# nfmoore/databricks-kubernetes-mlops-poc

Hardware: NVIDIA B200
Metric: rows/sec at batch=65536x23f (higher is better)
Workload: dtype u16 ranks + f64acc

## Files before the change

databricks_kubernetes_mlops_poc_b200/_cabi.py:

```python

from __future__ import annotations

import ctypes as C
import os

import numpy as np

ROW_WORDS = 24
ROW_BYTES = 96
PACKED_ROW_WORDS = 16
PACKED_ROW_BYTES = 64
ROWS_WORDS24 = 0
ROWS_PACKED64 = 1
ROWS_RANKED = 2
SCORED_DTYPE = np.dtype([("proba1", np.float32), ("label", np.int32)])
SCORED_FULL_DTYPE = np.dtype(
    [("proba1", np.float64), ("label", np.int32), ("is_outlier", np.int32), ("outlier_score", np.float32), ("reserved", np.int32)]
)
MOMENT_VALUES = ROW_WORDS * 3

_PKG_DIR = os.path.dirname(os.path.abspath(__file__))
LIB_PATH = os.path.join(_PKG_DIR, "lib", "libb200forest.so")

WALK_NAMES = {0: "smem", 1: "global"}
# ... 4 lines not shown
    """An engine call failed; the reference convention is "any exception -> HTTP 500"."""


class Info(C.Structure):
    _fields_ = [
        ("device", C.c_int32),
        ("sm_count", C.c_int32),
        ("agg_mode", C.c_int32),
        ("walk_mode", C.c_int32),
        ("n_trees", C.c_int32),
        ("n_groups", C.c_int32),
        ("max_depth", C.c_int32),
        ("n_cat", C.c_int32),
        ("n_num", C.c_int32),
        ("smem_bytes", C.c_int32),
        ("block_threads", C.c_int32),
        ("rows_per_warp", C.c_int32),
        ("forest_bytes", C.c_int64),
        ("launches", C.c_int64),
        ("launches_tile", C.c_int64),
        ("tile_min_rows", C.c_int64),
        ("tile_ok", C.c_int32),
        ("tile_resident", C.c_int32),
        ("packed_ok", C.c_int32),
        ("tile_warps", C.c_int32),
        ("launches_split", C.c_int64),
        ("split_max_rows", C.c_int64),
        ("outlier_trees", C.c_int32),
        ("rank_ok", C.c_int32),
        ("launches_rank", C.c_int64),
        ("rank_smem_bytes", C.c_int32),
        ("rank_row_bytes", C.c_int32),
        ("rank_stream", C.c_int32),
        ("reserved2", C.c_int32),
    ]


class RankInfo(C.Structure):

    _fields_ = [
        ("ok", C.c_int32),
        ("row_bytes", C.c_int32),
        ("cat_bytes", C.c_int32),
        ("n_cat", C.c_int32),
        ("n_num", C.c_int32),
        ("depth", C.c_int32),
        ("n_trees", C.c_int32),
        ("layout_bytes", C.c_int32),
        ("cat_shift", C.c_int32 * 16),
        ("cat_bits", C.c_int32 * 16),
        ("n_thresholds", C.c_int32 * 24),
        ("n_pairs", C.c_int32),
        ("pairs", C.c_uint32 * 128),
        ("why", C.c_char * 160),
    ]


class StrColumn(C.Structure):

    _fields_ = [
        ("offsets", C.c_void_p),
        ("data", C.c_void_p),
        ("validity", C.c_void_p),
        ("offset", C.c_int64),
        ("data_bytes", C.c_int64),
        ("offsets_are_64", C.c_int32),
        ("reserved", C.c_int32),
# ... 183 lines not shown
```

databricks_kubernetes_mlops_poc_b200/csrc/b2f_api.cu:

```cuda
#include <cuda_runtime.h>
#include <dlfcn.h>
#include <nccl.h>
#include <stdarg.h>
#include <stddef.h>
#include <stdio.h>
#include <stdlib.h>
#include <string.h>

#include <algorithm>
#include <string>
#include <thread>
#include <new>
#include <vector>

#include "../../include/b2f.h"
#include "feature_moments.cuh"
#include "forest_blob.h"
#include "forest_predict.cuh"
#include "forest_predict_tile.cuh"
#include "forest_predict_rank.cuh"
#include "forest_rank.h"
#include "json_rows.h"
#include "row_encoder.h"

#define B2F_VERSION_STR "b200forest 0.1.0 (sm_100a)"
#define B2F_STREAMS 4
#define B2F_TICKETS 256
#define B2F_CHUNK_ROWS 16384
#define B2F_FLUSH_BYTES (256ull << 20)

static thread_local char g_err[512] = "";

static int set_err(int code, const char *fmt, ...) {
    va_list ap;
    va_start(ap, fmt);
    vsnprintf(g_err, sizeof(g_err), fmt, ap);
    va_end(ap);
    return code;
}
#define CUDA_TRY(expr)                                                                         \
    do {                                                                                       \
        cudaError_t e_ = (expr);                                                               \
        if (e_ != cudaSuccess)                                                                 \
            return set_err(B2F_ECUDA, "%s failed: %s (%s:%d)", #expr, cudaGetErrorString(e_), __FILE__, __LINE__); \
    } while (0)
// ... 68 lines not shown
};

struct b2f_model {
    int device = 0;
    int sm_count = 0;
    int max_smem_optin = 0;
    KParams kp;
    b2f_blob_header hdr;
    int walk_mode = B2F_WALK_GLOBAL;
    int smem_bytes = 0;
    int rows_per_warp_max = 2;
    int64_t chunk_rows = B2F_CHUNK_ROWS;
    std::vector<int64_t> chunk_plan;
    bool tile_ok = false;
    TParams tp;
    void *d_tile_layout = nullptr;
    TPiece *d_tile_pieces = nullptr;
    int tile_smem_bytes = 0;
    int tile_cwarps = B2F_TILE_WARPS_MIN;
    int64_t tile_min_rows = 32768;
    int64_t tile_layout_bytes = 0;
    int64_t launches_tile = 0;
    int64_t launches_split = 0;
    int64_t split_max_rows = 0;
    bool packed_ok = false;
    b2f_ranker rk;
    bool rank_ok = false;
    RParams rp;
    void *d_rank_layout = nullptr;
    int rank_smem_bytes = 0;
    int rank_u = 4;
    bool rank_stream = false;
    int64_t launches_rank = 0;
    void *d_blob = nullptr;
    int64_t forest_bytes = 0;
    b2f_model *outlier = nullptr;
    Slot slots[B2F_STREAMS];
    cudaStream_t compute = nullptr;
    TicketRec tickets[B2F_TICKETS];
    uint64_t next_ticket = 1;
    uint64_t next_slot = 0;
    void *d_mom_rows = nullptr;
    int64_t mom_cap_rows = 0;
    double *d_mom_partials = nullptr;
    int mom_blocks = 0;
    unsigned int *d_mom_ticket = nullptr;
    double *d_mom_out = nullptr;
    double *d_gather = nullptr;
    int gather_cap = 0;
    void *d_flush = nullptr;
    ncclComm_t comm = nullptr;
    int nranks = 0;
    int rank = 0;
    int64_t launches = 0;
};

static int validate_blob(const uint8_t *blob, size_t nbytes, b2f_blob_header *hdr_out) {
    if (!blob || nbytes < sizeof(b2f_blob_header)) return set_err(B2F_EINVAL, "forest blob too small (%zu bytes)", nbytes);
    b2f_blob_header h;
    memcpy(&h, blob, sizeof(h));
    if (memcmp(h.magic, B2F_BLOB_MAGIC, 8) != 0) return set_err(B2F_EINVAL, "forest blob: bad magic");
    if (h.version != B2F_BLOB_VERSION) return set_err(B2F_EINVAL, "forest blob: version %u, expected %u", h.version, B2F_BLOB_VERSION);
    if (h.header_bytes != B2F_BLOB_HEADER_BYTES || h.row_words != B2F_ROW_WORDS)
        return set_err(B2F_EINVAL, "forest blob: header_bytes=%u row_words=%u unsupported", h.header_bytes, h.row_words);
    if (h.agg_mode != B2F_AGG_RF_MEAN && h.agg_mode != B2F_AGG_GBDT_LOGISTIC && h.agg_mode != B2F_AGG_IFOREST)
        return set_err(B2F_EINVAL, "forest blob: unknown agg_mode %u", h.agg_mode);
    if (h.n_trees == 0 || h.n_trees > B2F_MAX_TREES) return set_err(B2F_EINVAL, "forest blob: n_trees=%u out of range [1,%d]", h.n_trees, B2F_MAX_TREES);
    if (h.n_groups != (h.n_trees + 31) / 32) return set_err(B2F_EINVAL, "forest blob: n_groups=%u inconsistent with n_trees=%u", h.n_groups, h.n_trees);
    if (h.n_cat + h.n_num > B2F_SENTINEL_WORD) return set_err(B2F_EINVAL, "forest blob: n_cat+n_num=%u exceeds %u", h.n_cat + h.n_num, B2F_SENTINEL_WORD);
    if (h.total_bytes != nbytes) return set_err(B2F_EINVAL, "forest blob: total_bytes=%llu but %zu given", (unsigned long long)h.total_bytes, nbytes);
    if (h.groups_off < sizeof(h) || h.groups_off + (uint64_t)h.n_groups * sizeof(b2f_blob_group) > nbytes)
        return set_err(B2F_EINVAL, "forest blob: group table out of bounds");
    if (h.chunks_off % 256 || h.chunks_off + h.chunks_bytes > nbytes) return set_err(B2F_EINVAL, "forest blob: chunk area out of bounds");
    if (!(h.denom > 0.0)) return set_err(B2F_EINVAL, "forest blob: denom must be positive");
    const b2f_blob_group *gt = reinterpret_cast<const b2f_blob_group *>(blob + h.groups_off);
    uint64_t expect_off = 0;
    for (uint32_t g = 0; g < h.n_groups; ++g) {
        b2f_blob_group gr;
        memcpy(&gr, &gt[g], sizeof(gr));
        if (gr.chunk_off != expect_off || gr.n_slots == 0 || gr.n_leaf_slots == 0 ||
            gr.chunk_bytes != (gr.n_slots + gr.n_leaf_slots) * 256u || (uint64_t)gr.chunk_off + gr.chunk_bytes > h.chunks_bytes ||
            gr.n_slots >= (1u << 24) || gr.n_leaf_slots >= (1u << 24) || gr.n_trees == 0 || gr.n_trees > 32)
            return set_err(B2F_EINVAL, "forest blob: group %u descriptor invalid", g);
        expect_off += gr.chunk_bytes;
        const uint32_t *N = reinterpret_cast<const uint32_t *>(blob + h.chunks_off + gr.chunk_off);
        for (uint32_t s = 0; s < gr.n_slots; ++s)
            for (uint32_t l = 0; l < 32; ++l) {
                const uint32_t t = N[(s * 32 + l) * 2], m = N[(s * 32 + l) * 2 + 1];
// ... 206 lines not shown
        if (s < 2) return false;
        *n_slots = s;
    }
    return true;
}

template <int D, int U, bool ST, typename OutT>
static cudaError_t rank_set_attr(int bytes) {
    return cudaFuncSetAttribute(k_forest_predict_rank<D, U, ST, OutT>, cudaFuncAttributeMaxDynamicSharedMemorySize, bytes);
}
template <int U, bool ST>
static cudaError_t rank_set_attr_all(int depth, int bytes) {
    cudaError_t e = cudaSuccess;
#define RK_ATTR(DD)                                                        \
    case DD:                                                               \
        e = rank_set_attr<DD, U, ST, float>(bytes);                        \
        if (e == cudaSuccess) e = rank_set_attr<DD, U, ST, double>(bytes); \
        break;
    switch (depth) {
        RK_ATTR(1) RK_ATTR(2) RK_ATTR(3) RK_ATTR(4) RK_ATTR(5) RK_ATTR(6) RK_ATTR(7) RK_ATTR(8)
        default: e = cudaErrorInvalidValue;
    }
#undef RK_ATTR
    return e;
}

static int rank_init(b2f_model *m, const uint8_t *blob) {
    m->rank_ok = false;
    ranker_build(&m->rk, blob, m->hdr);
    if (!m->rk.ok) return B2F_OK;
    const char *off = getenv("B2F_RANK");
    if (off && !strcmp(off, "0")) return B2F_OK;
    const int64_t layout_bytes = (int64_t)m->rk.layout.size();
    const int64_t base = B2F_RANK_XS_BYTES  + (int64_t)B2F_RANK_PARTIALS * 32 * 8 + 256;
    int max_tiles = (int)std::min<int64_t>(B2F_RANK_MAX_TILES, ((int64_t)m->max_smem_optin - base - layout_bytes) / B2F_RANK_XS_BYTES);
    if (const char *mt = getenv("B2F_RANK_MAX_TILES")) max_tiles = std::min(max_tiles, std::max(1, atoi(mt)));
    m->rank_stream = max_tiles < 8;
    if (const char *fs = getenv("B2F_RANK_STREAM")) m->rank_stream = atoi(fs) != 0;
    int64_t forest_smem = layout_bytes;
    m->rank_u = 4;
    if (const char *ru = getenv("B2F_RANK_U")) m->rank_u = atoi(ru) == 8 ? 8 : 4;
    if (m->rank_stream) {
        m->rank_u = 4;
        const int64_t piece = 8 * (int64_t)m->rk.tree_stride;
        forest_smem = 2 * piece;
        max_tiles = (int)std::min<int64_t>(B2F_RANK_MAX_TILES, ((int64_t)m->max_smem_optin - base - forest_smem) / B2F_RANK_XS_BYTES);
        if (max_tiles < 4 || piece % 16) return B2F_OK;
    }
    CUDA_TRY(cudaMalloc(&m->d_rank_layout, (size_t)layout_bytes));
    CUDA_TRY(cudaMemcpy(m->d_rank_layout, m->rk.layout.data(), (size_t)layout_bytes, cudaMemcpyHostToDevice));
    RParams &rp = m->rp;
    memset(&rp, 0, sizeof(rp));
    rp.layout = static_cast<const uint8_t *>(m->d_rank_layout);
    rp.layout_bytes = (uint32_t)layout_bytes;
    rp.tree_stride = m->rk.tree_stride;
    rp.n_trees_padded = m->rk.n_trees_padded;
    rp.depth = m->rk.depth;
    rp.agg_mode = (int)m->hdr.agg_mode;
    rp.n_cat = m->rk.n_cat;
    rp.n_num = m->rk.n_num;
    rp.row_bytes = m->rk.row_bytes;
    rp.cat_bytes = m->rk.cat_bytes;
    rp.max_tiles = max_tiles;
    rp.groups_per_piece = 2;
    rp.piece_bytes = 8u * m->rk.tree_stride;
    rp.n_pieces = m->rk.n_trees_padded / 8;
    rp.init_raw = m->hdr.init_raw;
    rp.denom = m->hdr.denom;
    rp.threshold = m->hdr.threshold;
    rp.mul_two = 2u;
    rp.mul_64k = 65536u;
    rp.add_64k = 65535u;
    rp.n_pairs = (int)m->rk.pairs.size();
    for (int j = 0; j < 16; ++j) {
        rp.cat_shift[j] = (uint8_t)m->rk.cat_shift[j];
        rp.cat_bits[j] = (uint8_t)m->rk.cat_bits[j];
        rp.cat_start[j] = 0;
        rp.cat_mask[j] = 0ull;
    }
    for (int i = rp.n_pairs - 1; i >= 0; --i) {
        const uint32_t j = m->rk.pairs[i] >> 16, c = m->rk.pairs[i] & 0xFFFFu;
        rp.cat_start[j] = (uint8_t)i;
        rp.cat_mask[j] |= 1ull << c;
    }
    m->rank_smem_bytes = (int)(B2F_RANK_XS_BYTES + (int64_t)max_tiles * B2F_RANK_XS_BYTES + (int64_t)B2F_RANK_PARTIALS * 32 * 8 + forest_smem);
    if (m->rank_stream)
        CUDA_TRY((rank_set_attr_all<4, true>(rp.depth, m->rank_smem_bytes)));
    else
        CUDA_TRY(m->rank_u == 8 ? (rank_set_attr_all<8, false>(rp.depth, m->rank_smem_bytes)) : (rank_set_attr_all<4, false>(rp.depth, m->rank_smem_bytes)));
    m->rank_ok = true;
    return B2F_OK;
}

static bool kn_env_is(const char *v) {
    const char *kn = getenv("B2F_KERNEL");
    return kn && !strcmp(kn, v);
}

static int model_init_cuda(b2f_model *m, const uint8_t *blob, size_t nbytes) {
    CUDA_TRY(cudaSetDevice(m->device));
    cudaDeviceProp prop;
    CUDA_TRY(cudaGetDeviceProperties(&prop, m->device));
    if (prop.major < 10)
        return set_err(B2F_ENODEV, "device %d is sm_%d%d; this library is built for sm_100a (B200) only", m->device, prop.major, prop.minor);
    m->sm_count = prop.multiProcessorCount;
    CUDA_TRY(cudaDeviceGetAttribute(&m->max_smem_optin, cudaDevAttrMaxSharedMemoryPerBlockOptin, m->device));

    CUDA_TRY(cudaMalloc(&m->d_blob, nbytes));
    CUDA_TRY(cudaMemcpy(m->d_blob, blob, nbytes, cudaMemcpyHostToDevice));
    m->forest_bytes = (int64_t)m->hdr.chunks_bytes;

    KParams &kp = m->kp;
    memset(&kp, 0, sizeof(kp));
    kp.chunks = static_cast<const uint8_t *>(m->d_blob) + m->hdr.chunks_off;
    kp.n_groups = (int)m->hdr.n_groups;
    kp.agg_mode = (int)m->hdr.agg_mode;
    kp.n_cat = (int)m->hdr.n_cat;
// ... 135 lines not shown
    if (ndev < 0) return nullptr;
    if (device < 0 || device >= ndev) {
        set_err(B2F_EINVAL, "device %d out of range (have %d)", device, ndev);
        return nullptr;
    }
    b2f_model *m = new (std::nothrow) b2f_model();
    if (!m) {
        set_err(B2F_ENOMEM, "out of host memory");
        return nullptr;
    }
    m->device = device;
    if (validate_blob(static_cast<const uint8_t *>(forest_blob), nbytes, &m->hdr) != B2F_OK ||
        model_init_cuda(m, static_cast<const uint8_t *>(forest_blob), nbytes) != B2F_OK) {
        char keep[sizeof(g_err)];
        memcpy(keep, g_err, sizeof(keep));
        b2f_model_destroy(m);
        memcpy(g_err, keep, sizeof(keep));
        return nullptr;
    }
    return m;
}

extern "C" void b2f_model_destroy(b2f_model *m) {
    if (!m) return;
    cudaSetDevice(m->device);
    cudaDeviceSynchronize();
    if (m->outlier) b2f_model_destroy(m->outlier);
    if (m->comm && g_nccl.CommDestroy) g_nccl.CommDestroy(m->comm);
    for (int s = 0; s < B2F_STREAMS; ++s) {
        Slot &sl = m->slots[s];
        if (sl.d_rows) cudaFree(sl.d_rows);
        if (sl.d_proba) cudaFree(sl.d_proba);
        if (sl.d_label) cudaFree(sl.d_label);
        if (sl.stream) cudaStreamDestroy(sl.stream);
    }
    for (auto &t : m->tickets)
        for (auto &e : t.ev)
            if (e) cudaEventDestroy(e);
    if (m->compute) cudaStreamDestroy(m->compute);
    if (m->d_blob) cudaFree(m->d_blob);
    if (m->d_tile_layout) cudaFree(m->d_tile_layout);
    if (m->d_tile_pieces) cudaFree(m->d_tile_pieces);
    if (m->d_rank_layout) cudaFree(m->d_rank_layout);
    if (m->d_mom_rows) cudaFree(m->d_mom_rows);
    if (m->d_mom_partials) cudaFree(m->d_mom_partials);
    if (m->d_mom_ticket) cudaFree(m->d_mom_ticket);
    if (m->d_mom_out) cudaFree(m->d_mom_out);
    if (m->d_gather) cudaFree(m->d_gather);
    if (m->d_flush) cudaFree(m->d_flush);
    delete m;
}

static int pick_rows_per_warp(const b2f_model *m, int64_t n) {
    int r = m->rows_per_warp_max;
    const int64_t warps = (int64_t)m->sm_count * B2F_PREDICT_WARPS;
    while (r > 1 && n / r < warps) r >>= 1;
    return r;
}

extern "C" int b2f_model_info(const b2f_model *m, b2f_info *out) {
    if (!m || !out) return set_err(B2F_EINVAL, "null argument");
    memset(out, 0, sizeof(*out));
    out->device = m->device;
    out->sm_count = m->sm_count;
    out->agg_mode = (int)m->hdr.agg_mode;
    out->walk_mode = m->walk_mode;
    out->n_trees = (int)m->hdr.n_trees;
    out->n_groups = (int)m->hdr.n_groups;
    out->max_depth = (int)m->hdr.max_depth;
    out->n_cat = (int)m->hdr.n_cat;
    out->n_num = (int)m->hdr.n_num;
    out->smem_bytes = m->smem_bytes;
    out->block_threads = B2F_PREDICT_THREADS;
    out->rows_per_warp = m->rows_per_warp_max;
    out->forest_bytes = m->forest_bytes;
    out->launches = m->launches + (m->outlier ? m->outlier->launches : 0);
    out->launches_tile = m->launches_tile + (m->outlier ? m->outlier->launches_tile : 0);
    out->tile_min_rows = m->tile_min_rows;
    out->tile_ok = m->tile_ok ? 1 : 0;
    out->tile_resident = (m->tile_ok && m->tp.n_pieces <= m->tp.n_slots) ? 1 : 0;
    out->packed_ok = m->packed_ok ? 1 : 0;
    out->tile_warps = m->tile_ok ? m->tile_cwarps : 0;
    out->launches_split = m->launches_split;
    out->split_max_rows = m->split_max_rows;
    out->outlier_trees = m->outlier ? (int)m->outlier->hdr.n_trees : 0;
    out->rank_ok = m->rank_ok ? 1 : 0;
    out->launches_rank = m->launches_rank;
    out->rank_smem_bytes = m->rank_ok ? m->rank_smem_bytes : 0;
    out->rank_row_bytes = m->rk.row_bytes;
    out->rank_stream = (m->rank_ok && m->rank_stream) ? 1 : 0;
    return B2F_OK;
}

extern "C" int b2f_model_rank_info(const b2f_model *m, b2f_rank_info *out) {
    if (!m || !out) return set_err(B2F_EINVAL, "null argument");
    fill_rank_info(&m->rk, m->rank_ok, out);
    if (m->rk.ok && !m->rank_ok) snprintf(out->why, sizeof(out->why), "the rank layout (%zu bytes) does not stay resident in shared memory", m->rk.layout.size());
    return B2F_OK;
}

extern "C" void *b2f_pinned_alloc(size_t nbytes) {
    void *p = nullptr;
    cudaError_t e = cudaHostAlloc(&p, nbytes ? nbytes : 1, cudaHostAllocPortable);
    if (e != cudaSuccess) {
        set_err(B2F_ENOMEM, "cudaHostAlloc(%zu) failed: %s", nbytes, cudaGetErrorString(e));
        return nullptr;
    }
    return p;
}
extern "C" void b2f_pinned_free(void *p) {
    if (p) cudaFreeHost(p);
}

template <int R, bool SMEM, bool PACKED, typename OutT>
static cudaError_t launch_one(const b2f_model *m, cudaStream_t st, const void *rows, int64_t n, void *proba, int32_t *label, int ostride) {
    const int64_t n_batches = (n + R - 1) / R;
    int64_t ctas = std::min<int64_t>(m->sm_count, n_batches);
    if (ctas < 1) ctas = 1;
    k_forest_predict<R, SMEM, PACKED, OutT><<<(unsigned)ctas, B2F_PREDICT_THREADS, SMEM ? m->smem_bytes : 0, st>>>(
        m->kp, static_cast<const uint32_t *>(rows), (long long)n, static_cast<OutT *>(proba), label, ostride);
    return cudaGetLastError();
}

template <bool PACKED, typename OutT>
static cudaError_t launch_tile(const b2f_model *m, cudaStream_t st, const void *rows, int64_t n, void *proba, int32_t *label, int ostride) {
    const int64_t n_tiles = (n + B2F_TILE_ROWS - 1) / B2F_TILE_ROWS;
    const unsigned ctas = (unsigned)std::max<int64_t>(1, std::min<int64_t>(m->sm_count, n_tiles));
    k_forest_predict_tile<PACKED, OutT><<<ctas, (unsigned)(m->tile_cwarps + 1) * 32u, m->tile_smem_bytes, st>>>(m->tp, static_cast<const uint32_t *>(rows), (long long)n,
                                                                                           static_cast<OutT *>(proba), label, ostride);
    return cudaGetLastError();
}

template <bool PACKED, typename OutT>
static cudaError_t launch_split(const b2f_model *m, cudaStream_t st, const void *rows, int64_t n, void *proba, int32_t *label, int ostride) {
    constexpr int R = 2;
    const unsigned ctas = (unsigned)((n + R - 1) / R);
    k_forest_predict_split<R, PACKED, OutT><<<ctas, 32u * (unsigned)m->kp.n_groups, 0, st>>>(m->kp, static_cast<const uint32_t *>(rows), (long long)n,
                                                                                            static_cast<OutT *>(proba), label, ostride);
    return cudaGetLastError();
}

template <int D, int U, bool ST, typename OutT>
static cudaError_t launch_rank_du(const b2f_model *m, cudaStream_t st, const void *rows, int64_t n, void *proba, int32_t *label, int ostride) {
    const int64_t n_tiles = (n + 31) / 32;
    cudaLaunchConfig_t cfg = {};
    cfg.gridDim = dim3((unsigned)std::max<int64_t>(1, std::min<int64_t>(m->sm_count, n_tiles)));
    cfg.blockDim = dim3(B2F_RANK_THREADS);
    cfg.dynamicSmemBytes = (size_t)m->rank_smem_bytes;
    cfg.stream = st;
    cudaLaunchAttribute attr[1];
    attr[0].id = cudaLaunchAttributeProgrammaticStreamSerialization;
    attr[0].val.programmaticStreamSerializationAllowed = 1;
    static const bool no_pdl = getenv("B2F_NO_PDL") != nullptr;
    cfg.attrs = attr;
    cfg.numAttrs = no_pdl ? 0 : 1;
    return cudaLaunchKernelEx(&cfg, k_forest_predict_rank<D, U, ST, OutT>, m->rp, static_cast<const uint8_t *>(rows), (long long)n,
                              static_cast<OutT *>(proba), label, ostride);
}
template <typename OutT>
static cudaError_t launch_rank(const b2f_model *m, cudaStream_t st, const void *rows, int64_t n, void *proba, int32_t *label, int ostride) {
#define RK_CASE(DD)                                                                                                  \
    case DD:                                                                                                         \
        if (m->rank_stream) return launch_rank_du<DD, 4, true, OutT>(m, st, rows, n, proba, label, ostride);          \
        return m->rank_u == 8 ? launch_rank_du<DD, 8, false, OutT>(m, st, rows, n, proba, label, ostride)             \
                              : launch_rank_du<DD, 4, false, OutT>(m, st, rows, n, proba, label, ostride);
    switch (m->rp.depth) {
        RK_CASE(1) RK_CASE(2) RK_CASE(3) RK_CASE(4) RK_CASE(5) RK_CASE(6) RK_CASE(7) RK_CASE(8)
    }
#undef RK_CASE
    return cudaErrorInvalidValue;
}

static size_t row_bytes_of(const b2f_model *m, int fmt) {
    return fmt == B2F_ROWS_RANKED ? (size_t)m->rk.row_bytes : (fmt == B2F_ROWS_PACKED64 ? B2F_PACKED_ROW_BYTES : B2F_ROW_BYTES);
}

static int check_row_format(const b2f_model *m, int fmt) {
    if (fmt == B2F_ROWS_WORDS24) return B2F_OK;
    if (fmt == B2F_ROWS_RANKED) {
        if (!m->rank_ok)
            return set_err(B2F_EINVAL, "B2F_ROWS_RANKED is not available for this model (%s)",
                           m->rk.ok ? "its rank layout fits neither shared memory nor the streaming ring" : m->rk.why);
        return B2F_OK;
    }
    if (fmt != B2F_ROWS_PACKED64) return set_err(B2F_EINVAL, "unknown row format %d", fmt);
    if (!m->packed_ok) return set_err(B2F_EINVAL, "this model's schema does not fit the packed 64-byte row (needs exactly 9 categoricals with <= 126 categories, <= 14 numerics)");
    return B2F_OK;
}

static int launch_predict(b2f_model *m, cudaStream_t st, const void *rows_dev, int64_t n, int fmt, void *proba_dev, int f64, int32_t *label_dev,
                          int ostride = 1) {
    if (n <= 0) return B2F_OK;
    const bool pk = fmt == B2F_ROWS_PACKED64;
    cudaError_t e;
    if (fmt == B2F_ROWS_RANKED) {
        e = f64 ? launch_rank<double>(m, st, rows_dev, n, proba_dev, label_dev, ostride) : launch_rank<float>(m, st, rows_dev, n, proba_dev, label_dev, ostride);
        if (e != cudaSuccess) return set_err(B2F_ECUDA, "k_forest_predict_rank launch failed: %s", cudaGetErrorString(e));
        m->launches++;
        m->launches_rank++;
        return B2F_OK;
    }
    if (m->tile_ok && n >= m->tile_min_rows) {
        e = pk ? (f64 ? launch_tile<true, double>(m, st, rows_dev, n, proba_dev, label_dev, ostride) : launch_tile<true, float>(m, st, rows_dev, n, proba_dev, label_dev, ostride))
               : (f64 ? launch_tile<false, double>(m, st, rows_dev, n, proba_dev, label_dev, ostride) : launch_tile<false, float>(m, st, rows_dev, n, proba_dev, label_dev, ostride));
        if (e != cudaSuccess) return set_err(B2F_ECUDA, "k_forest_predict_tile launch failed: %s", cudaGetErrorString(e));
        m->launches++;
        m->launches_tile++;
        return B2F_OK;
    }
    if (n <= m->split_max_rows) {
        e = pk ? (f64 ? launch_split<true, double>(m, st, rows_dev, n, proba_dev, label_dev, ostride) : launch_split<true, float>(m, st, rows_dev, n, proba_dev, label_dev, ostride))
               : (f64 ? launch_split<false, double>(m, st, rows_dev, n, proba_dev, label_dev, ostride) : launch_split<false, float>(m, st, rows_dev, n, proba_dev, label_dev, ostride));
        if (e != cudaSuccess) return set_err(B2F_ECUDA, "k_forest_predict_split launch failed: %s", cudaGetErrorString(e));
        m->launches++;
        m->launches_split++;
        return B2F_OK;
    }
    const int r = pick_rows_per_warp(m, n);
    const bool sm = m->walk_mode == B2F_WALK_SMEM;
#define DISPATCH_T(RR, SM, PK)                                                                                      \
    (f64 ? launch_one<RR, SM, PK, double>(m, st, rows_dev, n, proba_dev, label_dev, ostride)                         \
         : launch_one<RR, SM, PK, float>(m, st, rows_dev, n, proba_dev, label_dev, ostride))
#define DISPATCH(RR) (sm ? (pk ? DISPATCH_T(RR, true, true) : DISPATCH_T(RR, true, false)) : (pk ? DISPATCH_T(RR, false, true) : DISPATCH_T(RR, false, false)))
    if (r == 4)
        e = DISPATCH(4);
    else if (r == 2)
        e = DISPATCH(2);
    else
        e = DISPATCH(1);
#undef DISPATCH
#undef DISPATCH_T
    if (e != cudaSuccess) return set_err(B2F_ECUDA, "k_forest_predict launch failed: %s", cudaGetErrorString(e));
// ... 600 lines not shown
```

databricks_kubernetes_mlops_poc_b200/csrc/forest_predict_rank.cuh:

```cuda
#pragma once
#include <cuda_runtime.h>
#include <stdint.h>

#include "forest_predict.cuh"
#include "forest_predict_tile.cuh"

#define B2F_RANK_THREADS 1024
#define B2F_RANK_WARPS 32
#define B2F_RANK_MAX_TILES 16
#define B2F_RANK_XS_BYTES 8192
#define B2F_RANK_PARTIALS (B2F_RANK_WARPS + B2F_RANK_MAX_TILES)

struct RParams {
    const uint8_t *layout;
    uint32_t layout_bytes;
    uint32_t tree_stride;
    int32_t n_trees_padded;
    int32_t depth;
    int32_t agg_mode;
    int32_t n_cat;
    int32_t n_num;
    int32_t row_bytes;
    int32_t cat_bytes;
    int32_t max_tiles;
    int32_t n_pieces;
    int32_t groups_per_piece;
    uint32_t piece_bytes;
    double init_raw;
    double denom;
    double threshold;
    uint32_t mul_two;
    uint32_t mul_64k;
    uint32_t add_64k;
    int32_t n_pairs;
    uint8_t cat_shift[16];
    uint8_t cat_bits[16];
    uint8_t cat_start[16];
    unsigned long long cat_mask[16];
};

__device__ __forceinline__ void pdl_launch_dependents() { asm volatile("griddepcontrol.launch_dependents;" ::: "memory"); }
__device__ __forceinline__ void pdl_wait() { asm volatile("griddepcontrol.wait;" ::: "memory"); }

__device__ __forceinline__ uint32_t lds_u16(uint32_t a) {
    uint32_t v;
    asm volatile("{ .reg .u16 h; ld.shared.u16 h, [%1]; cvt.u32.u16 %0, h; }" : "=r"(v) : "r"(a));
    return v;
}

template <int D, int U>
__device__ __forceinline__ void rank_walk_group(uint32_t t0, uint32_t tree_stride, uint32_t xs_lane, uint32_t m2, uint32_t m64k, uint32_t a64k,
                                                double &acc) {
    uint32_t at[U], k4[U], k8[U];
#pragma unroll
    for (int u = 0; u < U; ++u) {
        at[u] = t0 + u * tree_stride;
        k4[u] = 4u - at[u];
        k8[u] = 8u - at[u];
    }
#pragma unroll
    for (int d = 0; d < D; ++d) {
#pragma unroll
        for (int u = 0; u < U; ++u) {
            const uint32_t nw = lds32(at[u]);
            const uint32_t v = lds_u16(xs_lane | (nw & 0x1F82u));
            const uint32_t x = v * m64k + a64k;
            at[u] = at[u] * m2 + (x >= nw ? k8[u] : k4[u]);
        }
    }
#pragma unroll
    for (int u = 0; u < U; ++u) acc += lds_f64(at[u] + at[u] + k4[u] + 4u - (4u << D));
}

template <int D, int U, bool STREAM, typename OutT>
__global__ void __launch_bounds__(B2F_RANK_THREADS, 1)
    k_forest_predict_rank(const __grid_constant__ RParams p, const uint8_t *__restrict__ rows, long long n, OutT *__restrict__ proba,
                          int32_t *__restrict__ label, int ostride) {
    extern __shared__ __align__(128) uint8_t smem[];
    __shared__ __align__(8) uint64_t forest_bar[2];

    const int tid = threadIdx.x;
    const int lane = tid & 31;
    const int warp = tid >> 5;

    pdl_launch_dependents();

    const uint32_t pad = (B2F_RANK_XS_BYTES - (smem_addr(smem) & (B2F_RANK_XS_BYTES - 1u))) & (B2F_RANK_XS_BYTES - 1u);
    uint8_t *xs_all = smem + pad;
    double *partial = reinterpret_cast<double *>(xs_all + (size_t)p.max_tiles * B2F_RANK_XS_BYTES);
    uint8_t *forest = reinterpret_cast<uint8_t *>(partial + B2F_RANK_PARTIALS * 32);

    if (tid == 0) {
        mbar_init(&forest_bar[0], 1);
        mbar_init(&forest_bar[1], 1);
        fence_mbar_init();
        fence_proxy_async();
        if constexpr (!STREAM) {
            mbar_arrive_expect_tx(&forest_bar[0], p.layout_bytes);
            for (uint32_t o = 0; o < p.layout_bytes; o += B2F_BULK_PIECE) {
                const uint32_t part = min(B2F_BULK_PIECE, p.layout_bytes - o);
                tma_bulk_g2s(forest + o, p.layout + o, part, &forest_bar[0]);
            }
        }
    }
    auto issue_piece = [&](uint32_t k) {
        const uint32_t slot = k & 1u, piece = k % (uint32_t)p.n_pieces;
        mbar_arrive_expect_tx(&forest_bar[slot], p.piece_bytes);
        tma_bulk_g2s(forest + slot * p.piece_bytes, p.layout + (size_t)piece * p.piece_bytes, p.piece_bytes, &forest_bar[slot]);
    };

    const uint32_t n_tiles = (uint32_t)((n + 31) >> 5);
    const uint32_t tq = n_tiles / gridDim.x, tr = n_tiles % gridDim.x;
    const uint32_t tile0 = blockIdx.x * tq + min(blockIdx.x, tr), cta_tiles = tq + (blockIdx.x < tr ? 1u : 0u);
    const uint32_t n_rounds = (cta_tiles + (uint32_t)p.max_tiles - 1u) / (uint32_t)p.max_tiles;
    const int groups = p.n_trees_padded / U;
    const uint32_t forest_addr = smem_addr(forest);
    const uint32_t xs_addr = smem_addr(xs_all);
    bool forest_ready = false;

    pdl_wait();

    for (uint32_t round = 0; round < n_rounds; ++round) {
        const uint32_t rt0 = cta_tiles * round / n_rounds, rt1 = cta_tiles * (round + 1u) / n_rounds;
        const int T = (int)(rt1 - rt0);
        const long long row0 = (long long)(tile0 + rt0) * 32;
        const int n_rows = (int)min((long long)T * 32, n - row0);
        if (round > 0) __syncthreads();

        {
            const int items = T * 32 * 2;
            const int num_words = (p.n_num + 1) >> 1, hot_words = (p.n_pairs + 1) >> 1;
            for (int it = tid; it < items; it += B2F_RANK_THREADS) {
                const int part = it >= T * 32 ? 1 : 0, r = it - part * (T * 32);
                const uint32_t col = xs_addr + (uint32_t)(r >> 5) * B2F_RANK_XS_BYTES + (uint32_t)(r & 31) * 4u;
                const bool live = r < n_rows;
                const uint8_t *row = rows + (size_t)(row0 + (live ? r : 0)) * p.row_bytes;
                if (part == 0) {
                    const uint32_t *q = reinterpret_cast<const uint32_t *>(row + p.cat_bytes);
                    for (int w = 0; w < num_words; ++w) {
                        uint32_t v = live ? __ldg(q + w) : 0u;
                        if (2 * w + 1 >= p.n_num) v &= 0xFFFFu;
                        asm volatile("st.shared.u32 [%0], %1;" ::"r"(col + (uint32_t)w * 128u), "r"(v) : "memory");
                    }
                } else {
                    const uint32_t hot = col + (uint32_t)num_words * 128u;
                    for (int w = 0; w < hot_words; ++w) asm volatile("st.shared.u32 [%0], %1;" ::"r"(hot + (uint32_t)w * 128u), "r"(0u) : "memory");
                    if (live) {
                        unsigned long long cw = __ldg(reinterpret_cast<const uint32_t *>(row));
                        if (p.cat_bytes == 8) cw |= (unsigned long long)__ldg(reinterpret_cast<const uint32_t *>(row) + 1) << 32;
                        for (int j = 0; j < p.n_cat; ++j) {
                            const uint32_t code1 = (uint32_t)(cw >> p.cat_shift[j]) & ((1u << p.cat_bits[j]) - 1u);
                            const unsigned long long m = p.cat_mask[j];
                            if (code1 != 0u && code1 <= 64u && ((m >> (code1 - 1u)) & 1ull)) {
                                const uint32_t slot = (uint32_t)p.cat_start[j] + (uint32_t)__popcll(m & ((1ull << (code1 - 1u)) - 1ull));
                                asm volatile("st.shared.u16 [%0], %1;" ::"r"(hot + (slot >> 1) * 128u + (slot & 1u) * 2u), "h"((uint16_t)1) : "memory");
                            }
                        }
                    }
                }
            }
        }
        if constexpr (STREAM) {
            if (tid == 0) {
                issue_piece(round * (uint32_t)p.n_pieces);
                if (p.n_pieces > 1) issue_piece(round * (uint32_t)p.n_pieces + 1u);
            }
        }
        __syncthreads();
        if constexpr (!STREAM) {
            if (!forest_ready) {
                mbar_wait(&forest_bar[0], 0);
                forest_ready = true;
            }
        }

        if constexpr (STREAM) {
            const int GP = p.groups_per_piece;
            const bool mine = warp < T * GP;
            const uint32_t xs_lane = xs_addr + (uint32_t)(warp / GP) * B2F_RANK_XS_BYTES + (uint32_t)lane * 4u;
            const uint32_t g_off = (uint32_t)(warp % GP) * U * p.tree_stride;
            double acc = 0.0;
            for (int piece = 0; piece < p.n_pieces; ++piece) {
                const uint32_t k = round * (uint32_t)p.n_pieces + (uint32_t)piece;
                mbar_wait(&forest_bar[k & 1u], (k >> 1) & 1u);
                if (mine) rank_walk_group<D, U>(forest_addr + (k & 1u) * p.piece_bytes + g_off, p.tree_stride, xs_lane, p.mul_two, p.mul_64k, p.add_64k, acc);
                __syncthreads();
                if (tid == 0 && piece + 2 < p.n_pieces) issue_piece(k + 2u);
            }
            if (mine) partial[warp * 32 + lane] = acc;
            __syncthreads();
            for (int r = tid; r < n_rows; r += B2F_RANK_THREADS) {
                const int t = r >> 5, ln = r & 31;
                double s = p.agg_mode == B2F_AGG_GBDT_LOGISTIC ? p.init_raw : 0.0;
                for (int g = 0; g < GP; ++g) s += partial[(t * GP + g) * 32 + ln];
                double p1;
                int lab;
                aggregate(p.agg_mode, p.agg_mode == B2F_AGG_GBDT_LOGISTIC ? 0.0 : p.init_raw, p.denom, p.threshold, s, p1, lab);
                const long long row = row0 + r;
                if (proba) proba[row * ostride_p(ostride)] = (OutT)p1;
                if (label) label[row * ostride_l(ostride)] = lab;
            }
            continue;
        }

        {
            const int units = T * groups;
            int u = warp * units / B2F_RANK_WARPS;
            const int u_end = (warp + 1) * units / B2F_RANK_WARPS;
            while (u < u_end) {
                const int t = u / groups;
                const int g_end = min(groups, u_end - t * groups);
                const uint32_t xs_lane = xs_addr + (uint32_t)t * B2F_RANK_XS_BYTES + (uint32_t)lane * 4u;
                double acc = 0.0;
                for (int g = u - t * groups; g < g_end; ++g)
                    rank_walk_group<D, U>(forest_addr + (uint32_t)(g * U) * p.tree_stride, p.tree_stride, xs_lane, p.mul_two, p.mul_64k, p.add_64k, acc);
                partial[(warp + t) * 32 + lane] = acc;
                u = t * groups + g_end;
            }
        }
        __syncthreads();

        for (int r = tid; r < n_rows; r += B2F_RANK_THREADS) {
            const int t = r >> 5, ln = r & 31;
            const int units = T * groups;
            const int w_first = (int)(((uint32_t)(t * groups + 1) * B2F_RANK_WARPS + (uint32_t)units - 1u) / (uint32_t)units) - 1;
            const int w_last = (int)(((uint32_t)((t + 1) * groups) * B2F_RANK_WARPS + (uint32_t)units - 1u) / (uint32_t)units) - 1;
            double s = p.agg_mode == B2F_AGG_GBDT_LOGISTIC ? p.init_raw : 0.0;
            for (int w = w_first; w <= w_last; ++w)
                if ((w + 1) * units / B2F_RANK_WARPS > w * units / B2F_RANK_WARPS) s += partial[(w + t) * 32 + ln];
            double p1;
            int lab;
            aggregate(p.agg_mode, p.agg_mode == B2F_AGG_GBDT_LOGISTIC ? 0.0 : p.init_raw, p.denom, p.threshold, s, p1, lab);
            const long long row = row0 + r;
            if (proba) proba[row * ostride_p(ostride)] = (OutT)p1;
            if (label) label[row * ostride_l(ostride)] = lab;
        }
    }
    if constexpr (!STREAM) {
        if (!forest_ready) mbar_wait(&forest_bar[0], 0);
    }
}
```

include/b2f.h:

```cpp
#ifndef B2F_H
#define B2F_H

#include <stddef.h>
#include <stdint.h>

#ifdef __cplusplus
extern "C" {
#endif

#define B2F_ROW_WORDS 24
#define B2F_ROW_BYTES 96
#define B2F_PACKED_ROW_BYTES 64
#define B2F_MAX_TREES 1024
#define B2F_MOMENT_WORDS 3

#define B2F_ROWS_WORDS24 0
#define B2F_ROWS_PACKED64 1

#define B2F_ROWS_RANKED 2

#define B2F_OK 0
#define B2F_EINVAL (-1)
#define B2F_ECUDA (-2)
#define B2F_ENODEV (-3)
// ... 25 lines not shown
    float outlier_score;
    int32_t reserved;
} b2f_scored_full;

typedef struct b2f_info {
    int32_t device;
    int32_t sm_count;
    int32_t agg_mode;
    int32_t walk_mode;
    int32_t n_trees;
    int32_t n_groups;
    int32_t max_depth;
    int32_t n_cat;
    int32_t n_num;
    int32_t smem_bytes;
    int32_t block_threads;
    int32_t rows_per_warp;
    int64_t forest_bytes;
    int64_t launches;
    int64_t launches_tile;
    int64_t tile_min_rows;
    int32_t tile_ok;
    int32_t tile_resident;
    int32_t packed_ok;
    int32_t tile_warps;
    int64_t launches_split;
    int64_t split_max_rows;
    int32_t outlier_trees;
    int32_t rank_ok;
    int64_t launches_rank;
    int32_t rank_smem_bytes;
    int32_t rank_row_bytes;
    int32_t rank_stream;
    int32_t reserved2;
} b2f_info;

const char *b2f_version(void);
const char *b2f_last_error(void);
int b2f_device_count(void);

int b2f_blob_validate(const void *forest_blob, size_t nbytes);
b2f_model *b2f_model_create(const void *forest_blob, size_t nbytes, int device);
void b2f_model_destroy(b2f_model *m);
int b2f_model_info(const b2f_model *m, b2f_info *out);

typedef struct b2f_rank_info {
    int32_t ok;
    int32_t row_bytes;
    int32_t cat_bytes;
    int32_t n_cat, n_num;
    int32_t depth;
    int32_t n_trees;
    int32_t layout_bytes;
    int32_t cat_shift[16];
    int32_t cat_bits[16];
    int32_t n_thresholds[24];
    int32_t n_pairs;
    uint32_t pairs[128];
    char why[160];
} b2f_rank_info;
typedef struct b2f_ranker b2f_ranker;
b2f_ranker *b2f_ranker_create(const void *forest_blob, size_t nbytes);
void b2f_ranker_destroy(b2f_ranker *r);
int b2f_ranker_info(const b2f_ranker *r, b2f_rank_info *out);
const float *b2f_ranker_thresholds(const b2f_ranker *r, int k, int32_t *count);
const void *b2f_ranker_layout(const b2f_ranker *r, int64_t *nbytes);
int b2f_ranker_rank_rows(const b2f_ranker *r, const void *rows, int64_t n, int row_format, void *ranked_out, int threads);
// ... 129 lines not shown
```

Before: 3.722 billion.

## Defer PDL wait past tree walk, add packed head records, track output hazards

Moves the griddepcontrol.wait in the ranked forest kernel from before row staging to after the tree walk, so a dependent launch can stage rows and walk trees while the previous kernel finishes. To keep this safe, the host records each stream's recent output ranges and turns PDL off when the new input rows overlap prior outputs. It also adds a packed per-group head table with the root and level-1 nodes of each tree, read with vector shared loads, to cut scattered loads in the first two levels. A compile-time tracing hook is included. The trade-offs are extra shared memory for the head table, which can lower max_tiles, and a host mutex plus hash map lookup on every launch.

```diff
diff --git a/databricks_kubernetes_mlops_poc_b200/_cabi.py b/databricks_kubernetes_mlops_poc_b200/_cabi.py
--- a/databricks_kubernetes_mlops_poc_b200/_cabi.py
+++ b/databricks_kubernetes_mlops_poc_b200/_cabi.py
@@ -60,7 +60,7 @@
         ("rank_smem_bytes", C.c_int32),
         ("rank_row_bytes", C.c_int32),
         ("rank_stream", C.c_int32),
-        ("reserved2", C.c_int32),
+        ("rank_last_pdl", C.c_int32),
     ]
 
 
diff --git a/databricks_kubernetes_mlops_poc_b200/csrc/b2f_api.cu b/databricks_kubernetes_mlops_poc_b200/csrc/b2f_api.cu
--- a/databricks_kubernetes_mlops_poc_b200/csrc/b2f_api.cu
+++ b/databricks_kubernetes_mlops_poc_b200/csrc/b2f_api.cu
@@ -8,9 +8,12 @@
 #include <string.h>
 
 #include <algorithm>
+#include <deque>
+#include <mutex>
 #include <string>
 #include <thread>
 #include <new>
+#include <unordered_map>
 #include <vector>
 
 #include "../../include/b2f.h"
@@ -145,6 +148,10 @@
     int rank_u = 4;
     bool rank_stream = false;
     int64_t launches_rank = 0;
+    bool rank_last_pdl = false;
+#ifdef B2F_RANK_TRACE
+    unsigned long long *d_rank_trace = nullptr;
+#endif
     void *d_blob = nullptr;
     int64_t forest_bytes = 0;
     b2f_model *outlier = nullptr;
@@ -167,6 +174,40 @@
     int rank = 0;
     int64_t launches = 0;
 };
+
+struct RankWrites {
+    uintptr_t p0, p1, l0, l1;
+};
+static std::mutex g_rank_writes_mu;
+static std::unordered_map<cudaStream_t, std::deque<RankWrites>> g_rank_writes;
+
+static bool rank_launch_pdl(cudaStream_t st, int sm_count, const void *rows, size_t rows_bytes, const void *proba, size_t psz, const int32_t *label,
+                            int64_t n, int ostride) {
+    static const bool no_pdl = getenv("B2F_NO_PDL") != nullptr;
+    const int64_t ps = ostride & 0xffff, ls = (ostride >> 16) ? (ostride >> 16) : ps;
+    RankWrites w;
+    w.p0 = reinterpret_cast<uintptr_t>(proba);
+    w.p1 = proba ? w.p0 + (size_t)((n - 1) * ps + 1) * psz : w.p0;
+    w.l0 = reinterpret_cast<uintptr_t>(label);
+    w.l1 = label ? w.l0 + (size_t)((n - 1) * ls + 1) * sizeof(int32_t) : w.l0;
+    const uintptr_t r0 = reinterpret_cast<uintptr_t>(rows), r1 = r0 + rows_bytes;
+    std::lock_guard<std::mutex> lk(g_rank_writes_mu);
+    std::deque<RankWrites> &chain = g_rank_writes[st];
+    bool pdl = !no_pdl;
+    for (const RankWrites &c : chain)
+        if ((c.p0 < r1 && r0 < c.p1) || (c.l0 < r1 && r0 < c.l1)) {
+            pdl = false;
+            break;
+        }
+    if (!pdl) chain.clear();
+    chain.push_back(w);
+    while (chain.size() > 2 * (size_t)sm_count + 1) chain.pop_front();
+    return pdl;
+}
+static void rank_forget_stream(cudaStream_t st) {
+    std::lock_guard<std::mutex> lk(g_rank_writes_mu);
+    g_rank_writes.erase(st);
+}
 
 static int validate_blob(const uint8_t *blob, size_t nbytes, b2f_blob_header *hdr_out) {
     if (!blob || nbytes < sizeof(b2f_blob_header)) return set_err(B2F_EINVAL, "forest blob too small (%zu bytes)", nbytes);
@@ -439,29 +480,47 @@
     const char *off = getenv("B2F_RANK");
     if (off && !strcmp(off, "0")) return B2F_OK;
     const int64_t layout_bytes = (int64_t)m->rk.layout.size();
+    const int64_t head_bytes = (int64_t)m->rk.n_trees_padded * 12;
     const int64_t base = B2F_RANK_XS_BYTES  + (int64_t)B2F_RANK_PARTIALS * 32 * 8 + 256;
-    int max_tiles = (int)std::min<int64_t>(B2F_RANK_MAX_TILES, ((int64_t)m->max_smem_optin - base - layout_bytes) / B2F_RANK_XS_BYTES);
+    int max_tiles = (int)std::min<int64_t>(B2F_RANK_MAX_TILES, ((int64_t)m->max_smem_optin - base - layout_bytes - head_bytes) / B2F_RANK_XS_BYTES);
     if (const char *mt = getenv("B2F_RANK_MAX_TILES")) max_tiles = std::min(max_tiles, std::max(1, atoi(mt)));
     m->rank_stream = max_tiles < 8;
     if (const char *fs = getenv("B2F_RANK_STREAM")) m->rank_stream = atoi(fs) != 0;
-    int64_t forest_smem = layout_bytes;
+    int64_t forest_smem = layout_bytes + head_bytes;
     m->rank_u = 4;
     if (const char *ru = getenv("B2F_RANK_U")) m->rank_u = atoi(ru) == 8 ? 8 : 4;
+    std::vector<uint8_t> dev_layout(m->rk.layout);
     if (m->rank_stream) {
         m->rank_u = 4;
         const int64_t piece = 8 * (int64_t)m->rk.tree_stride;
         forest_smem = 2 * piece;
         max_tiles = (int)std::min<int64_t>(B2F_RANK_MAX_TILES, ((int64_t)m->max_smem_optin - base - forest_smem) / B2F_RANK_XS_BYTES);
         if (max_tiles < 4 || piece % 16) return B2F_OK;
-    }
-    CUDA_TRY(cudaMalloc(&m->d_rank_layout, (size_t)layout_bytes));
-    CUDA_TRY(cudaMemcpy(m->d_rank_layout, m->rk.layout.data(), (size_t)layout_bytes, cudaMemcpyHostToDevice));
+    } else {
+        const int U = m->rank_u, n_nodes = 1 << m->rk.depth;
+        std::vector<uint32_t> head((size_t)head_bytes / 4, 0u);
+        for (int t = 0; t < m->rk.n_trees_padded; ++t) {
+            const uint32_t *nodes = reinterpret_cast<const uint32_t *>(m->rk.layout.data() + (size_t)t * m->rk.tree_stride);
+            uint32_t *g = head.data() + (size_t)(t / U) * 3 * U;
+            g[t % U] = nodes[0];
+            if (n_nodes > 2) {
+                g[U + 2 * (t % U)] = nodes[1];
+                g[U + 2 * (t % U) + 1] = nodes[2];
+            }
+        }
+        dev_layout.resize((size_t)(layout_bytes + head_bytes));
+        memcpy(dev_layout.data() + layout_bytes, head.data(), (size_t)head_bytes);
+    }
+    CUDA_TRY(cudaMalloc(&m->d_rank_layout, dev_layout.size()));
+    CUDA_TRY(cudaMemcpy(m->d_rank_layout, dev_layout.data(), dev_layout.size(), cudaMemcpyHostToDevice));
     RParams &rp = m->rp;
     memset(&rp, 0, sizeof(rp));
     rp.layout = static_cast<const uint8_t *>(m->d_rank_layout);
-    rp.layout_bytes = (uint32_t)layout_bytes;
+    rp.layout_bytes = (uint32_t)dev_layout.size();
     rp.tree_stride = m->rk.tree_stride;
     rp.n_trees_padded = m->rk.n_trees_padded;
+    rp.n_groups = (m->rk.n_trees + m->rank_u - 1) / m->rank_u;
+    rp.head_off = (uint32_t)layout_bytes;
     rp.depth = m->rk.depth;
     rp.agg_mode = (int)m->hdr.agg_mode;
     rp.n_cat = m->rk.n_cat;
@@ -490,6 +549,11 @@
         rp.cat_start[j] = (uint8_t)i;
         rp.cat_mask[j] |= 1ull << c;
     }
+#ifdef B2F_RANK_TRACE
+    const size_t trace_bytes = (size_t)B2F_RANK_TRACE_LAUNCHES * m->sm_count * B2F_RANK_TRACE_WORDS * sizeof(unsigned long long);
+    CUDA_TRY(cudaMalloc(&m->d_rank_trace, trace_bytes));
+    CUDA_TRY(cudaMemset(m->d_rank_trace, 0, trace_bytes));
+#endif
     m->rank_smem_bytes = (int)(B2F_RANK_XS_BYTES + (int64_t)max_tiles * B2F_RANK_XS_BYTES + (int64_t)B2F_RANK_PARTIALS * 32 * 8 + forest_smem);
     if (m->rank_stream)
         CUDA_TRY((rank_set_attr_all<4, true>(rp.depth, m->rank_smem_bytes)));
@@ -691,16 +755,25 @@
         if (sl.d_rows) cudaFree(sl.d_rows);
         if (sl.d_proba) cudaFree(sl.d_proba);
         if (sl.d_label) cudaFree(sl.d_label);
-        if (sl.stream) cudaStreamDestroy(sl.stream);
+        if (sl.stream) {
+            rank_forget_stream(sl.stream);
+            cudaStreamDestroy(sl.stream);
+        }
     }
     for (auto &t : m->tickets)
         for (auto &e : t.ev)
             if (e) cudaEventDestroy(e);
-    if (m->compute) cudaStreamDestroy(m->compute);
+    if (m->compute) {
+        rank_forget_stream(m->compute);
+        cudaStreamDestroy(m->compute);
+    }
     if (m->d_blob) cudaFree(m->d_blob);
     if (m->d_tile_layout) cudaFree(m->d_tile_layout);
     if (m->d_tile_pieces) cudaFree(m->d_tile_pieces);
     if (m->d_rank_layout) cudaFree(m->d_rank_layout);
+#ifdef B2F_RANK_TRACE
+    if (m->d_rank_trace) cudaFree(m->d_rank_trace);
+#endif
     if (m->d_mom_rows) cudaFree(m->d_mom_rows);
     if (m->d_mom_partials) cudaFree(m->d_mom_partials);
     if (m->d_mom_ticket) cudaFree(m->d_mom_ticket);
@@ -748,6 +821,7 @@
     out->rank_smem_bytes = m->rank_ok ? m->rank_smem_bytes : 0;
     out->rank_row_bytes = m->rk.row_bytes;
     out->rank_stream = (m->rank_ok && m->rank_stream) ? 1 : 0;
+    out->rank_last_pdl = m->rank_last_pdl ? 1 : 0;
     return B2F_OK;
 }
 
@@ -800,7 +874,7 @@
 }
 
 template <int D, int U, bool ST, typename OutT>
-static cudaError_t launch_rank_du(const b2f_model *m, cudaStream_t st, const void *rows, int64_t n, void *proba, int32_t *label, int ostride) {
+static cudaError_t launch_rank_du(const b2f_model *m, cudaStream_t st, const void *rows, int64_t n, void *proba, int32_t *label, int ostride, bool pdl) {
     const int64_t n_tiles = (n + 31) / 32;
     cudaLaunchConfig_t cfg = {};
     cfg.gridDim = dim3((unsigned)std::max<int64_t>(1, std::min<int64_t>(m->sm_count, n_tiles)));
@@ -810,19 +884,37 @@
     cudaLaunchAttribute attr[1];
     attr[0].id = cudaLaunchAttributeProgrammaticStreamSerialization;
     attr[0].val.programmaticStreamSerializationAllowed = 1;
-    static const bool no_pdl = getenv("B2F_NO_PDL") != nullptr;
     cfg.attrs = attr;
-    cfg.numAttrs = no_pdl ? 0 : 1;
-    return cudaLaunchKernelEx(&cfg, k_forest_predict_rank<D, U, ST, OutT>, m->rp, static_cast<const uint8_t *>(rows), (long long)n,
+    cfg.numAttrs = pdl ? 1 : 0;
+#ifdef B2F_RANK_TRACE
+    RParams rp = m->rp;
+    rp.trace = m->d_rank_trace + (size_t)(m->launches_rank % B2F_RANK_TRACE_LAUNCHES) * m->sm_count * B2F_RANK_TRACE_WORDS;
+#else
+    const RParams &rp = m->rp;
+#endif
+    return cudaLaunchKernelEx(&cfg, k_forest_predict_rank<D, U, ST, OutT>, rp, static_cast<const uint8_t *>(rows), (long long)n,
                               static_cast<OutT *>(proba), label, ostride);
 }
+
+#ifdef B2F_RANK_TRACE
+extern "C" int64_t b2f_rank_trace_read(b2f_model *m, unsigned long long *out, int32_t *launch_slots, int32_t *ctas_per_launch) {
+    if (!m || !out || !m->d_rank_trace) return -1;
+    if (cudaSetDevice(m->device) != cudaSuccess || cudaDeviceSynchronize() != cudaSuccess) return -1;
+    if (cudaMemcpy(out, m->d_rank_trace, (size_t)B2F_RANK_TRACE_LAUNCHES * m->sm_count * B2F_RANK_TRACE_WORDS * sizeof(unsigned long long),
+                   cudaMemcpyDeviceToHost) != cudaSuccess)
+        return -1;
+    *launch_slots = B2F_RANK_TRACE_LAUNCHES;
+    *ctas_per_launch = m->sm_count;
+    return m->launches_rank;
+}
+#endif
 template <typename OutT>
-static cudaError_t launch_rank(const b2f_model *m, cudaStream_t st, const void *rows, int64_t n, void *proba, int32_t *label, int ostride) {
+static cudaError_t launch_rank(const b2f_model *m, cudaStream_t st, const void *rows, int64_t n, void *proba, int32_t *label, int ostride, bool pdl) {
 #define RK_CASE(DD)                                                                                                  \
     case DD:                                                                                                         \
-        if (m->rank_stream) return launch_rank_du<DD, 4, true, OutT>(m, st, rows, n, proba, label, ostride);          \
-        return m->rank_u == 8 ? launch_rank_du<DD, 8, false, OutT>(m, st, rows, n, proba, label, ostride)             \
-                              : launch_rank_du<DD, 4, false, OutT>(m, st, rows, n, proba, label, ostride);
+        if (m->rank_stream) return launch_rank_du<DD, 4, true, OutT>(m, st, rows, n, proba, label, ostride, pdl);     \
+        return m->rank_u == 8 ? launch_rank_du<DD, 8, false, OutT>(m, st, rows, n, proba, label, ostride, pdl)        \
+                              : launch_rank_du<DD, 4, false, OutT>(m, st, rows, n, proba, label, ostride, pdl);
     switch (m->rp.depth) {
         RK_CASE(1) RK_CASE(2) RK_CASE(3) RK_CASE(4) RK_CASE(5) RK_CASE(6) RK_CASE(7) RK_CASE(8)
     }
@@ -853,10 +945,13 @@
     const bool pk = fmt == B2F_ROWS_PACKED64;
     cudaError_t e;
     if (fmt == B2F_ROWS_RANKED) {
-        e = f64 ? launch_rank<double>(m, st, rows_dev, n, proba_dev, label_dev, ostride) : launch_rank<float>(m, st, rows_dev, n, proba_dev, label_dev, ostride);
+        const bool pdl = rank_launch_pdl(st, m->sm_count, rows_dev, (size_t)n * (size_t)m->rk.row_bytes, proba_dev, f64 ? sizeof(double) : sizeof(float), label_dev, n, ostride);
+        e = f64 ? launch_rank<double>(m, st, rows_dev, n, proba_dev, label_dev, ostride, pdl)
+                : launch_rank<float>(m, st, rows_dev, n, proba_dev, label_dev, ostride, pdl);
         if (e != cudaSuccess) return set_err(B2F_ECUDA, "k_forest_predict_rank launch failed: %s", cudaGetErrorString(e));
         m->launches++;
         m->launches_rank++;
+        m->rank_last_pdl = pdl;
         return B2F_OK;
     }
     if (m->tile_ok && n >= m->tile_min_rows) {
diff --git a/databricks_kubernetes_mlops_poc_b200/csrc/forest_predict_rank.cuh b/databricks_kubernetes_mlops_poc_b200/csrc/forest_predict_rank.cuh
--- a/databricks_kubernetes_mlops_poc_b200/csrc/forest_predict_rank.cuh
+++ b/databricks_kubernetes_mlops_poc_b200/csrc/forest_predict_rank.cuh
@@ -16,6 +16,8 @@
     uint32_t layout_bytes;
     uint32_t tree_stride;
     int32_t n_trees_padded;
+    int32_t n_groups;
+    uint32_t head_off;
     int32_t depth;
     int32_t agg_mode;
     int32_t n_cat;
@@ -37,7 +39,35 @@
     uint8_t cat_bits[16];
     uint8_t cat_start[16];
     unsigned long long cat_mask[16];
+#ifdef B2F_RANK_TRACE
+    unsigned long long *trace;
+#endif
 };
+
+#define B2F_RANK_TRACE_WORDS 8
+#define B2F_RANK_TRACE_LAUNCHES 256
+enum { RT_SMID, RT_ENTRY, RT_FOREST, RT_WAIT, RT_STAGED, RT_WALKED, RT_EXIT };
+#ifdef B2F_RANK_TRACE
+__device__ __forceinline__ unsigned long long rank_trace_now() {
+    unsigned long long t;
+    asm volatile("mov.u64 %0, %%globaltimer;" : "=l"(t));
+    return t;
+}
+__device__ __forceinline__ unsigned long long rank_trace_smid() {
+    uint32_t s;
+    asm volatile("mov.u32 %0, %%smid;" : "=r"(s));
+    return s;
+}
+#define RANK_TRACE(i)                                                                                                       \
+    do {                                                                                                                    \
+        if (threadIdx.x == 0)                                                                                               \
+            p.trace[(size_t)blockIdx.x * B2F_RANK_TRACE_WORDS + (i)] = (i) == RT_SMID ? rank_trace_smid() : rank_trace_now(); \
+    } while (0)
+#else
+#define RANK_TRACE(i) \
+    do {              \
+    } while (0)
+#endif
 
 __device__ __forceinline__ void pdl_launch_dependents() { asm volatile("griddepcontrol.launch_dependents;" ::: "memory"); }
 __device__ __forceinline__ void pdl_wait() { asm volatile("griddepcontrol.wait;" ::: "memory"); }
@@ -48,18 +78,11 @@
     return v;
 }
 
-template <int D, int U>
-__device__ __forceinline__ void rank_walk_group(uint32_t t0, uint32_t tree_stride, uint32_t xs_lane, uint32_t m2, uint32_t m64k, uint32_t a64k,
-                                                double &acc) {
-    uint32_t at[U], k4[U], k8[U];
-#pragma unroll
-    for (int u = 0; u < U; ++u) {
-        at[u] = t0 + u * tree_stride;
-        k4[u] = 4u - at[u];
-        k8[u] = 8u - at[u];
-    }
-#pragma unroll
-    for (int d = 0; d < D; ++d) {
+template <int D0, int D, int U>
+__device__ __forceinline__ void rank_walk_levels(uint32_t (&at)[U], const uint32_t (&k4)[U], const uint32_t (&k8)[U], uint32_t xs_lane, uint32_t m2,
+                                                 uint32_t m64k, uint32_t a64k, double &acc) {
+#pragma unroll
+    for (int d = D0; d < D; ++d) {
 #pragma unroll
         for (int u = 0; u < U; ++u) {
             const uint32_t nw = lds32(at[u]);
@@ -70,6 +93,47 @@
     }
 #pragma unroll
     for (int u = 0; u < U; ++u) acc += lds_f64(at[u] + at[u] + k4[u] + 4u - (4u << D));
+}
+
+template <int D, int U>
+__device__ __forceinline__ void rank_walk_group(uint32_t t0, uint32_t tree_stride, uint32_t xs_lane, uint32_t m2, uint32_t m64k, uint32_t a64k,
+                                                double &acc) {
+    uint32_t at[U], k4[U], k8[U];
+#pragma unroll
+    for (int u = 0; u < U; ++u) {
+        at[u] = t0 + u * tree_stride;
+        k4[u] = 4u - at[u];
+        k8[u] = 8u - at[u];
+    }
+    rank_walk_levels<0, D, U>(at, k4, k8, xs_lane, m2, m64k, a64k, acc);
+}
+
+template <int D, int U>
+__device__ __forceinline__ void rank_walk_group_head(uint32_t t0, uint32_t hd, uint32_t tree_stride, uint32_t xs_lane, uint32_t m2, uint32_t m64k,
+                                                     uint32_t a64k, double &acc) {
+    static_assert(U % 4 == 0, "head records are read 4 words at a time");
+    uint32_t hw[3 * U];
+#pragma unroll
+    for (int q = 0; q < 3 * U / 4; ++q)
+        asm volatile("ld.shared.v4.u32 {%0, %1, %2, %3}, [%4];"
+                     : "=r"(hw[4 * q]), "=r"(hw[4 * q + 1]), "=r"(hw[4 * q + 2]), "=r"(hw[4 * q + 3])
+                     : "r"(hd + 16u * q));
+    uint32_t at[U], k4[U], k8[U];
+#pragma unroll
+    for (int u = 0; u < U; ++u) {
+        at[u] = t0 + u * tree_stride;
+        k4[u] = 4u - at[u];
+        k8[u] = 8u - at[u];
+        const uint32_t r = hw[u];
+        const bool c0 = lds_u16(xs_lane | (r & 0x1F82u)) * m64k + a64k >= r;
+        at[u] = at[u] * m2 + (c0 ? k8[u] : k4[u]);
+        if constexpr (D >= 2) {
+            const uint32_t n1 = c0 ? hw[U + 2 * u + 1] : hw[U + 2 * u];
+            const bool c1 = lds_u16(xs_lane | (n1 & 0x1F82u)) * m64k + a64k >= n1;
+            at[u] = at[u] * m2 + (c1 ? k8[u] : k4[u]);
+        }
+    }
+    rank_walk_levels<(D >= 2 ? 2 : 1), D, U>(at, k4, k8, xs_lane, m2, m64k, a64k, acc);
 }
 
 template <int D, int U, bool STREAM, typename OutT>
@@ -84,6 +148,8 @@
     const int warp = tid >> 5;
 
     pdl_launch_dependents();
+    RANK_TRACE(RT_SMID);
+    RANK_TRACE(RT_ENTRY);
 
     const uint32_t pad = (B2F_RANK_XS_BYTES - (smem_addr(smem) & (B2F_RANK_XS_BYTES - 1u))) & (B2F_RANK_XS_BYTES - 1u);
     uint8_t *xs_all = smem + pad;
@@ -113,12 +179,11 @@
     const uint32_t tq = n_tiles / gridDim.x, tr = n_tiles % gridDim.x;
     const uint32_t tile0 = blockIdx.x * tq + min(blockIdx.x, tr), cta_tiles = tq + (blockIdx.x < tr ? 1u : 0u);
     const uint32_t n_rounds = (cta_tiles + (uint32_t)p.max_tiles - 1u) / (uint32_t)p.max_tiles;
-    const int groups = p.n_trees_padded / U;
+    const int groups = p.n_groups;
     const uint32_t forest_addr = smem_addr(forest);
     const uint32_t xs_addr = smem_addr(xs_all);
+    const uint32_t head_addr = forest_addr + p.head_off;
     bool forest_ready = false;
-
-    pdl_wait();
 
     for (uint32_t round = 0; round < n_rounds; ++round) {
         const uint32_t rt0 = cta_tiles * round / n_rounds, rt1 = cta_tiles * (round + 1u) / n_rounds;
@@ -167,11 +232,13 @@
             }
         }
         __syncthreads();
+        RANK_TRACE(RT_STAGED);
         if constexpr (!STREAM) {
             if (!forest_ready) {
                 mbar_wait(&forest_bar[0], 0);
                 forest_ready = true;
             }
+            RANK_TRACE(RT_FOREST);
         }
 
         if constexpr (STREAM) {
@@ -189,6 +256,9 @@
             }
             if (mine) partial[warp * 32 + lane] = acc;
             __syncthreads();
+            RANK_TRACE(RT_WALKED);
+            pdl_wait();
+            RANK_TRACE(RT_WAIT);
             for (int r = tid; r < n_rows; r += B2F_RANK_THREADS) {
                 const int t = r >> 5, ln = r & 31;
                 double s = p.agg_mode == B2F_AGG_GBDT_LOGISTIC ? p.init_raw : 0.0;
@@ -213,12 +283,16 @@
                 const uint32_t xs_lane = xs_addr + (uint32_t)t * B2F_RANK_XS_BYTES + (uint32_t)lane * 4u;
                 double acc = 0.0;
                 for (int g = u - t * groups; g < g_end; ++g)
-                    rank_walk_group<D, U>(forest_addr + (uint32_t)(g * U) * p.tree_stride, p.tree_stride, xs_lane, p.mul_two, p.mul_64k, p.add_64k, acc);
+                    rank_walk_group_head<D, U>(forest_addr + (uint32_t)(g * U) * p.tree_stride, head_addr + (uint32_t)g * (12u * U), p.tree_stride,
+                                               xs_lane, p.mul_two, p.mul_64k, p.add_64k, acc);
                 partial[(warp + t) * 32 + lane] = acc;
                 u = t * groups + g_end;
             }
         }
         __syncthreads();
+        RANK_TRACE(RT_WALKED);
+        pdl_wait();
+        RANK_TRACE(RT_WAIT);
 
         for (int r = tid; r < n_rows; r += B2F_RANK_THREADS) {
             const int t = r >> 5, ln = r & 31;
@@ -239,4 +313,5 @@
     if constexpr (!STREAM) {
         if (!forest_ready) mbar_wait(&forest_bar[0], 0);
     }
-}
+    RANK_TRACE(RT_EXIT);
+}
diff --git a/include/b2f.h b/include/b2f.h
--- a/include/b2f.h
+++ b/include/b2f.h
@@ -81,7 +81,7 @@
     int32_t rank_smem_bytes;
     int32_t rank_row_bytes;
     int32_t rank_stream;
-    int32_t reserved2;
+    int32_t rank_last_pdl;
 } b2f_info;
 
 const char *b2f_version(void);
```

Result: faster. 4.086 billion, median of 6 (+9.8%).
